# gunrock/mini

Hardware: AMD Instinct MI355X
Metric: MTEPS (million traversed edges/sec) BFS advance+filter, RMAT-22 (higher is better)
Workload: dtype int32

## Files before the change

### include/mgx/bfs_fused_mini.hpp

```cpp
#pragma once
#include "bfs_fused.hpp"
#include "bfs_fused_chain.hpp"

namespace mgx {

constexpr int BFS_MINI_WGS = 64;
constexpr int BFS_MINI_LCAP = 4096;
constexpr int BFS_MINI_WCAP = 8192;
constexpr u32 BFS_MINI_EDGES_LATE = 131072;
constexpr u32 BFS_MINI_EDGES_EARLY = 32768;
constexpr u32 BFS_MINI_SHORT_ROWS = 65536;
constexpr size_t bfs_mini_lds_bytes() {
  return (size_t)(2 * BFS_MINI_LCAP + 4) * 4 + (size_t)BFS_MINI_WCAP * 4 + 64 * 8 + 256;
}

__device__ __forceinline__ bool bfs_level_is_mini(const bfs_fused_args_t& a, const bfs_ctrl_t* c, int slot) {
  if (a.mode != 0 || c->lazy_slot == slot) return false;
  const u64 cur = c->cursor[slot % 3], lcur = c->lcursor[slot % 3];
  const u64 E = (cur & BFS_EMASK) + c->ledges[slot % 3];
  const bool late = c->reached * 4ull >= (u64)(u32)a.n;
  return (lcur >> BFS_VSHIFT) <= (u64)BFS_MINI_LCAP && (cur >> BFS_VSHIFT) <= (u64)BFS_MINI_SHORT_ROWS &&
         E <= (u64)(late ? BFS_MINI_EDGES_LATE : BFS_MINI_EDGES_EARLY);
}

template <int NT>
__global__ __launch_bounds__(NT) void k_bfs_mini(bfs_fused_args_t a, int arg) {
  constexpr int NW = NT / WAVE;
  constexpr u64 CNT1 = 1ull << 40;
  constexpr u64 DEGMASK = CNT1 - 1ull;
  extern __shared__ __attribute__((aligned(16))) char smem[];
  u32* const s_loff = (u32*)smem;
  u32* const s_lrow = s_loff + BFS_MINI_LCAP + 4;
  u32* const s_win = s_lrow + BFS_MINI_LCAP;
  u64* const s_scan = (u64*)(s_win + BFS_MINI_WCAP);
  __shared__ int s_cnt, s_maxdeg;
  __shared__ u64 s_base[2];
  __shared__ u32 s_long_true;
  bfs_ctrl_t* const c = a.ctrl;
  int slot, level;
  bfs_resolve(c, arg, slot, level);
  if (c->done) return;
  const u64 cur = c->cursor[slot % 3], lcur = c->lcursor[slot % 3];
  const u64 ledges = c->ledges[slot % 3];
  const int nf_s = (int)(cur >> BFS_VSHIFT), nf_l = (int)(lcur >> BFS_VSHIFT);
  const u32 Es = (u32)(cur & BFS_EMASK), Rl = (u32)(lcur & BFS_EMASK);
  const int in = slot & 1, out = (slot + 1) & 1;
  const bool first_thread = blockIdx.x == 0 && threadIdx.x == 0;
  if (nf_s + nf_l == 0) {
    if (first_thread) {
      c->cursor[(slot + 2) % 3] = 0; c->lcursor[(slot + 2) % 3] = 0; c->ledges[(slot + 2) % 3] = 0;
      if (level < 64) c->stamp[level] = __builtin_amdgcn_s_memrealtime();
      if (!c->done) { c->done = 1; c->levels = level; }
    }
    return;
  }
  const long long gtid = (long long)blockIdx.x * NT + threadIdx.x, gthreads = (long long)gridDim.x * NT;
  if (!bfs_level_is_mini(a, c, slot)) {
    const bool lazy = c->lazy_slot == slot;
    const bool fb = c->fb_slot == slot;
    if (!lazy) {
      for (long long i = gtid; i < nf_s; i += gthreads) { a.fr_row[out][i] = a.fr_row[in][i]; a.fr_off[out][i] = a.fr_off[in][i]; }
      for (long long i = gtid; i < nf_l; i += gthreads) { a.lq_row[out][i] = a.lq_row[in][i]; a.lq_off[out][i] = a.lq_off[in][i]; }
    }
    __syncthreads();
    if (threadIdx.x == 0) {
      __threadfence();
      if (atomicAdd(&c->mini_blocks[slot & 3], 1u) == gridDim.x - 1u) {
        c->mini_blocks[slot & 3] = 0u;
        c->cursor[(slot + 1) % 3] = cur; c->lcursor[(slot + 1) % 3] = lcur; c->ledges[(slot + 1) % 3] = ledges;
        c->cursor[(slot + 2) % 3] = 0; c->lcursor[(slot + 2) % 3] = 0; c->ledges[(slot + 2) % 3] = 0;
        c->slot_level[(slot + 1) & 3] = level;
        c->flush_count[(slot + 1) & 1] = 0;
        bfs_slot_marks_clear(a, slot + 1);
        if (lazy) c->lazy_slot = slot + 1;
        if (fb) c->fb_slot = slot + 1;
      }
    }
    return;
  }
  if (first_thread) {
    const u64 E = (u64)Es + ledges;
    c->cursor[(slot + 2) % 3] = 0; c->lcursor[(slot + 2) % 3] = 0; c->ledges[(slot + 2) % 3] = 0;
    if (level < 64) c->stamp[level] = __builtin_amdgcn_s_memrealtime();
    if (level < BFS_MAX_TRACE) c->trace[level] = ((u64)(nf_s + nf_l) << BFS_VSHIFT) | E;
    c->sum_edges += E;
    c->sum_frontier += (u64)(nf_s + nf_l);
    c->sum_long_edges += ledges;
    c->sum_long_vertices += (u64)nf_l;
    c->push_levels += 1;
    c->small_levels += 1;
    c->mini_slots += 1;
    c->slots += 1;
    c->slot_level[(slot + 1) & 3] = level + 1;
    c->flush_count[(slot + 1) & 1] = 0;
    bfs_slot_marks_clear(a, slot + 1);
    c->fb_slot = -1;
  }
  const int lane = lane_id();
  const int wave = threadIdx.x / WAVE;
  const u32 long_min = a.long_min > 0 ? (u32)a.long_min : 0xFFFFFFFFu;
  const int new_label = level + 1;
  for (int i = threadIdx.x; i < nf_l; i += NT) { s_loff[i] = a.lq_off[in][i]; s_lrow[i] = a.lq_row[in][i]; }
  if (threadIdx.x == 0) { s_loff[nf_l] = Rl; s_cnt = 0; s_maxdeg = 0; }
  __syncthreads();

  u64* const cur_s = &c->cursor[(slot + 1) % 3];
  u64* const cur_l = &c->lcursor[(slot + 1) % 3];
  u32* __restrict__ const out_row_s = a.fr_row[out];
  u32* __restrict__ const out_off_s = a.fr_off[out];
  u32* __restrict__ const out_row_l = a.lq_row[out];
  u32* __restrict__ const out_off_l = a.lq_off[out];
  int found = 0;

  auto flush = [&]() {
    __syncthreads();
    const int W = s_cnt;
    for (int first = 0; first < W; first += NT) {
      const int i = first + (int)threadIdx.x;
      u32 ro = 0, deg = 0;
      if (i < W) {
        const u32 v = s_win[i];
        const bfs_u32x2 ext = *(const bfs_u32x2*)(a.row_offsets + v);
        ro = ext.x; deg = ext.y - ext.x;
        a.labels[a.old_of_new ? a.old_of_new[v] : (int)v] = new_label;
      }
      const bool is_long = deg >= long_min;
      const u64 add_s = (!is_long && deg) ? (CNT1 | (u64)deg) : 0ull;
      const u64 add_l = is_long ? (CNT1 | (u64)bfs_lq_pad(deg)) : 0ull;
      if (threadIdx.x == 0) s_long_true = 0;
      u64 tot_s, tot_l;
      const u64 ex_s = block_exclusive_sum_lean<NW>(add_s, s_scan, &tot_s);
      const u64 ex_l = block_exclusive_sum_lean<NW>(add_l, s_scan, &tot_l);
      const u32 lt = wave_sum(is_long ? deg : 0u);
      if (lane == 0 && lt) atomicAdd(&s_long_true, lt);
      __syncthreads();
      if (threadIdx.x == 0) {
        s_base[0] = (tot_s >> 40) ? atomicAdd(cur_s, ((tot_s >> 40) << BFS_VSHIFT) | (tot_s & DEGMASK)) : 0ull;
        s_base[1] = (tot_l >> 40) ? atomicAdd(cur_l, ((tot_l >> 40) << BFS_VSHIFT) | (tot_l & DEGMASK)) : 0ull;
        if (tot_l >> 40) atomicAdd(&c->ledges[(slot + 1) % 3], (u64)s_long_true);
      }
      __syncthreads();
      if (deg) {
        const u64 b = is_long ? s_base[1] : s_base[0];
        const u64 at = is_long ? ex_l : ex_s;
        const u64 pos = (b >> BFS_VSHIFT) + (at >> 40);
        (is_long ? out_row_l : out_row_s)[pos] = ro;
        (is_long ? out_off_l : out_off_s)[pos] = (u32)((b & BFS_EMASK) + (at & DEGMASK)) | (is_long ? (deg & 63u) : 0u);
      }
      __syncthreads();
    }
    if (threadIdx.x == 0) s_cnt = 0;
    __syncthreads();
  };
  auto visit = [&](bool act, u32 d) {
    bool win = false;
    if (act) {
      const u32 bit = 1u << (d & 31u);
      const u32 seen = a.visited[d >> 5];
      if (!(seen & bit)) win = !(atomicOr(a.visited + (d >> 5), bit) & bit);
    }
    const u64 bal = __ballot(win);
    if (bal) {
      int at = 0;
      if (lane == 0) at = atomicAdd(&s_cnt, __popcll(bal));
      at = __builtin_amdgcn_readfirstlane(at);
      if (win) { s_win[at + rank_in_mask(bal)] = d; ++found; }
    }
  };

  {
    const u32 U = Rl >> 6;
    const u32 Wt = (u32)gridDim.x * NW, w0 = (u32)blockIdx.x * NW + (u32)wave;
    const u32 iters = (U + Wt - 1u) / Wt;
    for (u32 t = 0; t < iters; ++t) {
      const u32 u = w0 + t * Wt;
      bool act = false;
      u32 d = 0;
      if (u < U) {
        const u32 r0 = u << 6;
        int lo = 0, hi = nf_l;
        while (hi - lo > 1) { const int mid = (lo + hi) >> 1; if ((s_loff[mid] & ~63u) <= r0) lo = mid; else hi = mid; }
        const u32 e0 = s_loff[lo];
        const u32 deg = bfs_lq_degree(e0, s_loff[lo + 1]);
        const u32 rank = r0 - (e0 & ~63u) + (u32)lane;
        act = rank < deg;
        if (act) d = (u32)a.col_indices[s_lrow[lo] + rank];
      }
      visit(act, d);
      __syncthreads();
      const int cnt_now = s_cnt;
      __syncthreads();
      if (cnt_now > BFS_MINI_WCAP - NT) flush();
    }
  }
  if (nf_s > 0 && (u64)Es >= 4ull * (u64)nf_s) {
    const u32* __restrict__ fr_row = a.fr_row[in];
    const u32* __restrict__ fr_off = a.fr_off[in];
    const u32 iters = (Es + (u32)gthreads - 1u) / (u32)gthreads;
    for (u32 t = 0; t < iters; ++t) {
      const u64 r64 = (u64)gtid + (u64)t * (u64)gthreads;
      const bool act = r64 < (u64)Es;
      const u32 r = act ? (u32)r64 : 0u;
      int lo = 0, hi = nf_s;
      while (hi - lo > 1) { const int mid = (lo + hi) >> 1; if (fr_off[mid] <= r) lo = mid; else hi = mid; }
      const u32 d = act ? (u32)a.col_indices[fr_row[lo] + (r - fr_off[lo])] : 0u;
      visit(act, d);
      __syncthreads();
      const int cnt_now = s_cnt;
      __syncthreads();
      if (cnt_now > BFS_MINI_WCAP - NT) flush();
    }
  } else
  {
    const u32* __restrict__ fr_row = a.fr_row[in];
    const u32* __restrict__ fr_off = a.fr_off[in];
    const u32 iters = ((u32)nf_s + (u32)gthreads - 1u) / (u32)gthreads;
    for (u32 t = 0; t < iters; ++t) {
      const long long i = gtid + (long long)t * gthreads;
      u32 row = 0, deg = 0;
      if (i < nf_s) {
        const u32 e0 = fr_off[i], e1 = (i + 1 < nf_s) ? fr_off[i + 1] : Es;
        row = fr_row[i];
        deg = e1 - e0;
      }
      int wmax = (int)deg;
#pragma unroll
      for (int sh = WAVE / 2; sh > 0; sh >>= 1) { const int o = __shfl_xor(wmax, sh, WAVE); wmax = o > wmax ? o : wmax; }
      if (lane == 0 && wmax) atomicMax(&s_maxdeg, wmax);
      __syncthreads();
      const u32 kmax = (u32)s_maxdeg;
      for (u32 k = 0; k < kmax; ++k) {
        const bool act = k < deg;
        const u32 d = act ? (u32)a.col_indices[row + k] : 0u;
        visit(act, d);
        __syncthreads();
        const int cnt_now = s_cnt;
        __syncthreads();
        if (cnt_now > BFS_MINI_WCAP - NT) flush();
      }
      __syncthreads();
      if (threadIdx.x == 0) s_maxdeg = 0;
      __syncthreads();
    }
  }
  flush();
  found = (int)wave_sum((u32)found);
  if (lane == 0 && found) atomicAdd(&c->reached_mini, (u64)found);
}

}
```

Measured before the change: 449,400.

## Batch four frontier rows per thread in mini BFS and widen mini thresholds

The thread-per-row path of the single-launch mini BFS kernel now handles four frontier rows per thread per step. It issues the column and visited-word loads for all four before doing the atomic claims, which gives more memory-level parallelism and fewer barriers per edge. The flush threshold is lowered so the winner buffer still fits four claims per thread. The mini path's edge and row limits are also raised, so more BFS levels take the mini kernel. The risks are more divergence from skewed row degrees across the four rows, extra register pressure, and big levels running on a small grid.

```diff
diff --git a/include/mgx/bfs_fused_mini.hpp b/include/mgx/bfs_fused_mini.hpp
--- a/include/mgx/bfs_fused_mini.hpp
+++ b/include/mgx/bfs_fused_mini.hpp
@@ -7,9 +7,10 @@
 constexpr int BFS_MINI_WGS = 64;
 constexpr int BFS_MINI_LCAP = 4096;
 constexpr int BFS_MINI_WCAP = 8192;
-constexpr u32 BFS_MINI_EDGES_LATE = 131072;
-constexpr u32 BFS_MINI_EDGES_EARLY = 32768;
-constexpr u32 BFS_MINI_SHORT_ROWS = 65536;
+constexpr u32 BFS_MINI_EDGES_LATE = 524288;
+constexpr u32 BFS_MINI_EDGES_EARLY = 40960;
+constexpr u32 BFS_MINI_SHORT_ROWS = 524288;
+constexpr int BFS_MINI_ROWS_PT = 4;
 constexpr size_t bfs_mini_lds_bytes() {
   return (size_t)(2 * BFS_MINI_LCAP + 4) * 4 + (size_t)BFS_MINI_WCAP * 4 + 64 * 8 + 256;
 }
@@ -152,11 +153,10 @@
     if (threadIdx.x == 0) s_cnt = 0;
     __syncthreads();
   };
-  auto visit = [&](bool act, u32 d) {
+  auto claim = [&](bool act, u32 d, u32 seen) {
     bool win = false;
     if (act) {
       const u32 bit = 1u << (d & 31u);
-      const u32 seen = a.visited[d >> 5];
       if (!(seen & bit)) win = !(atomicOr(a.visited + (d >> 5), bit) & bit);
     }
     const u64 bal = __ballot(win);
@@ -167,6 +167,7 @@
       if (win) { s_win[at + rank_in_mask(bal)] = d; ++found; }
     }
   };
+  auto visit = [&](bool act, u32 d) { claim(act, d, act ? a.visited[d >> 5] : 0u); };
 
   {
     const u32 U = Rl >> 6;
@@ -212,31 +213,41 @@
     }
   } else
   {
+    constexpr int RT = BFS_MINI_ROWS_PT;
     const u32* __restrict__ fr_row = a.fr_row[in];
     const u32* __restrict__ fr_off = a.fr_off[in];
     const u32 iters = ((u32)nf_s + (u32)gthreads - 1u) / (u32)gthreads;
-    for (u32 t = 0; t < iters; ++t) {
-      const long long i = gtid + (long long)t * gthreads;
-      u32 row = 0, deg = 0;
-      if (i < nf_s) {
-        const u32 e0 = fr_off[i], e1 = (i + 1 < nf_s) ? fr_off[i + 1] : Es;
-        row = fr_row[i];
-        deg = e1 - e0;
-      }
-      int wmax = (int)deg;
+    for (u32 t = 0; t < iters; t += RT) {
+      u32 row[RT], deg[RT];
+      int wmax = 0;
+#pragma unroll
+      for (int q = 0; q < RT; ++q) {
+        const long long i = gtid + (long long)(t + q) * gthreads;
+        row[q] = 0; deg[q] = 0;
+        if (i < nf_s) {
+          const u32 e0 = fr_off[i], e1 = (i + 1 < nf_s) ? fr_off[i + 1] : Es;
+          row[q] = fr_row[i];
+          deg[q] = e1 - e0;
+        }
+        wmax = (int)deg[q] > wmax ? (int)deg[q] : wmax;
+      }
 #pragma unroll
       for (int sh = WAVE / 2; sh > 0; sh >>= 1) { const int o = __shfl_xor(wmax, sh, WAVE); wmax = o > wmax ? o : wmax; }
       if (lane == 0 && wmax) atomicMax(&s_maxdeg, wmax);
       __syncthreads();
       const u32 kmax = (u32)s_maxdeg;
       for (u32 k = 0; k < kmax; ++k) {
-        const bool act = k < deg;
-        const u32 d = act ? (u32)a.col_indices[row + k] : 0u;
-        visit(act, d);
+        u32 d[RT], seen[RT];
+#pragma unroll
+        for (int q = 0; q < RT; ++q) d[q] = k < deg[q] ? (u32)a.col_indices[row[q] + k] : 0u;
+#pragma unroll
+        for (int q = 0; q < RT; ++q) seen[q] = k < deg[q] ? a.visited[d[q] >> 5] : 0u;
+#pragma unroll
+        for (int q = 0; q < RT; ++q) claim(k < deg[q], d[q], seen[q]);
         __syncthreads();
         const int cnt_now = s_cnt;
         __syncthreads();
-        if (cnt_now > BFS_MINI_WCAP - NT) flush();
+        if (cnt_now > BFS_MINI_WCAP - RT * NT) flush();
       }
       __syncthreads();
       if (threadIdx.x == 0) s_maxdeg = 0;
```

Result: slower. 433,900, median of 2 (-3.5%).
